# clearml/clearml-serving

Measured on AMD Instinct MI355X. Metric: requests/sec + p50 latency, ResNet-50 & BERT-base dyn-batch, 1/2/4/8 MI355X, higher is better.
Workload: dtype bf16; 1 GPU; model=resnet50+bert-base, global_batch=512, seq_len=128, image=3x224x224, parallelism=dp1, max_batch_size=64, outputs_consumed=16673280

## Files before the change

### clearml_serving_amd/models/resnet.py

```python

import torch
import torch.nn as nn
import torch.nn.functional as F

from .. import ops
from . import register_arch


class FoldedConv(nn.Module):

    def __init__(self, cin, cout, k, stride=1, padding=0, relu=False):
        super().__init__()
        self.conv = nn.Conv2d(cin, cout, k, stride=stride, padding=padding,
                              bias=True)
        self.relu = relu

    def forward(self, x):
        c = self.conv
        if (c.kernel_size == (3, 3) and c.stride == (1, 1)
                and c.padding == (1, 1)
                and ops.conv3x3_supported(x, c.weight)):
            return ops.conv3x3_nhwc(x, c.weight, c.bias, relu=self.relu)
        y = c(x)
        if self.relu:
            y = F.relu(y)
        return y


class StemConv(nn.Module):

    def __init__(self, cin, cout, k, stride, padding, relu=True):
        super().__init__()
        self.conv = nn.Conv2d(cin, cout, k, stride=stride, padding=padding,
                              bias=True)
        self.relu = relu
        self.k, self.stride, self.padding = k, stride, padding

    def forward(self, x):
        if not x.is_cuda:
            y = self.conv(x)
            return F.relu(y) if self.relu else y
        n, c, h, w = x.shape
        oh = (h + 2 * self.padding - self.k) // self.stride + 1
        ow = (w + 2 * self.padding - self.k) // self.stride + 1
        cols = F.unfold(x.contiguous(), self.k, stride=self.stride,
                        padding=self.padding)
        flat = cols.transpose(1, 2).reshape(-1, c * self.k * self.k)
        wmat = self.conv.weight.reshape(self.conv.out_channels, -1)
        y = torch.nn.functional.linear(flat, wmat, self.conv.bias)
        if self.relu:
            y = torch.relu(y)
        return y.view(n, oh, ow, self.conv.out_channels) \
            .permute(0, 3, 1, 2)


def fold_bn_into_conv(conv: nn.Conv2d, bn: nn.BatchNorm2d) -> None:
    with torch.no_grad():
        inv_std = torch.rsqrt(bn.running_var + bn.eps)
        scale = bn.weight * inv_std
        conv.weight.mul_(scale[:, None, None, None])
        bias = conv.bias.data if conv.bias is not None else torch.zeros_like(bn.bias)
        conv.bias = nn.Parameter(bn.bias + (bias - bn.running_mean) * scale)


class Bottleneck(nn.Module):
    expansion = 4

    def __init__(self, cin, width, stride=1, downsample=None):
        super().__init__()
        cout = width * self.expansion
        self.conv1 = FoldedConv(cin, width, 1, relu=True)
        self.conv2 = FoldedConv(width, width, 3, stride=stride, padding=1,
                                relu=True)
        self.conv3 = FoldedConv(width, cout, 1, relu=False)
        self.downsample = downsample

    def forward(self, x):
        identity = x if self.downsample is None else self.downsample(x)
        y = self.conv1(x)
        y = self.conv2(y)
        y = self.conv3.conv(y)
        return ops.bias_relu_add(y, residual=identity)


class ResNet(nn.Module):
    def __init__(self, layers=(3, 4, 6, 3), num_classes=1000):
        super().__init__()
        self.stem = FoldedConv(3, 64, 7, stride=2, padding=3, relu=True)
        self.maxpool = nn.MaxPool2d(3, stride=2, padding=1)
        self.inplanes = 64
        self.layer1 = self._make_layer(64, layers[0], stride=1)
        self.layer2 = self._make_layer(128, layers[1], stride=2)
        self.layer3 = self._make_layer(256, layers[2], stride=2)
        self.layer4 = self._make_layer(512, layers[3], stride=2)
        self.fc = nn.Linear(512 * Bottleneck.expansion, num_classes)
        self._init_weights()

    def _make_layer(self, width, blocks, stride):
        downsample = None
        cout = width * Bottleneck.expansion
        if stride != 1 or self.inplanes != cout:
            downsample = FoldedConv(self.inplanes, cout, 1, stride=stride)
        layers = [Bottleneck(self.inplanes, width, stride, downsample)]
        self.inplanes = cout
        for _ in range(1, blocks):
            layers.append(Bottleneck(self.inplanes, width))
        return nn.Sequential(*layers)

    def _init_weights(self):
        for m in self.modules():
            if isinstance(m, nn.Conv2d):
                nn.init.kaiming_normal_(m.weight, mode="fan_out",
                                        nonlinearity="relu")
                if m.bias is not None:
                    nn.init.zeros_(m.bias)

    def forward(self, x):
        x = x.contiguous(memory_format=torch.channels_last)
        x = self.stem(x)
        x = self.maxpool(x)
        x = self.layer1(x)
        x = self.layer2(x)
        x = self.layer3(x)
        x = self.layer4(x)
        x = x.mean(dim=(2, 3))
        return self.fc(x)


@register_arch("resnet50")
def resnet50(num_classes: int = 1000) -> ResNet:
    return ResNet(layers=(3, 4, 6, 3), num_classes=num_classes).to(
        memory_format=torch.channels_last)


@register_arch("resnet101")
def resnet101(num_classes: int = 1000) -> ResNet:
    return ResNet(layers=(3, 4, 23, 3), num_classes=num_classes).to(
        memory_format=torch.channels_last)
```

### clearml_serving_amd/ops/__init__.py

```python

import importlib.machinery
import importlib.util
import math
import os
from typing import Optional, Tuple

import torch

_ext = None
_ext_error: Optional[str] = None
_FORCE_EAGER = os.environ.get("CLEARML_SERVING_AMD_FORCE_EAGER") == "1"


def _try_load_ext() -> None:
    global _ext, _ext_error
    if _ext is not None or _ext_error is not None:
        return
    so_path = os.path.join(os.path.dirname(__file__), "_hip_ops.so")
    if not os.path.exists(so_path):
        _ext_error = "extension not built ({} missing)".format(so_path)
        return
    try:
        loader = importlib.machinery.ExtensionFileLoader("_hip_ops", so_path)
        spec = importlib.util.spec_from_loader("_hip_ops", loader)
        mod = importlib.util.module_from_spec(spec)
        loader.exec_module(mod)
        _ext = mod
    except Exception as ex:
        _ext_error = "failed loading {}: {}".format(so_path, ex)


_try_load_ext()


def has_extension() -> bool:
    return _ext is not None


def _require_ext(opname: str):
    if _FORCE_EAGER:
        return None
    if _ext is None:
        raise RuntimeError(
            "clearml_serving_amd HIP extension required for GPU op '{}' but "
            "not loaded: {}. Build it with __graft_entry__.build() "
            "(hipcc --offload-arch=gfx950).".format(opname, _ext_error)
        )
    return _ext


def extension_or_none():
    return _ext


def layernorm(
    x: torch.Tensor, weight: torch.Tensor, bias: torch.Tensor,
    eps: float = 1e-5, residual: Optional[torch.Tensor] = None,
) -> torch.Tensor:
    if x.is_cuda:
        ext = _require_ext("layernorm")
        if ext is not None:
            return ext.layernorm(x, weight, bias, eps, residual)
    if residual is not None:
        x = x + residual
    return torch.nn.functional.layer_norm(
        x.float(), (x.shape[-1],), weight.float(), bias.float(), eps
    ).to(x.dtype)


def rmsnorm(
    x: torch.Tensor, weight: torch.Tensor, eps: float = 1e-6,
    residual: Optional[torch.Tensor] = None,
) -> torch.Tensor:
    if x.is_cuda:
        ext = _require_ext("rmsnorm")
        if ext is not None:
            return ext.rmsnorm(x, weight, eps, residual)
    xf = x.float()
    if residual is not None:
        xf = xf + residual.float()
        residual.copy_(xf.to(residual.dtype))
    out = xf * torch.rsqrt(xf.pow(2).mean(-1, keepdim=True) + eps)
    return (out * weight.float()).to(x.dtype)


def bias_gelu(x: torch.Tensor, bias: Optional[torch.Tensor] = None) -> torch.Tensor:
    if x.is_cuda:
        ext = _require_ext("bias_gelu")
        if ext is not None:
            return ext.bias_gelu(x, bias)
    if bias is not None:
        x = x + bias
    return torch.nn.functional.gelu(x.float()).to(x.dtype)


def bias_relu_add(
    x: torch.Tensor, bias: Optional[torch.Tensor] = None,
    residual: Optional[torch.Tensor] = None,
) -> torch.Tensor:
    if x.is_cuda:
        ext = _require_ext("bias_relu_add")
        if ext is not None:
            return ext.bias_relu_add(x, bias, residual)
    if bias is not None:
        x = x + bias
    if residual is not None:
        x = x + residual
    return torch.relu(x)


def silu_mul(gate: torch.Tensor, up: torch.Tensor) -> torch.Tensor:
    if gate.is_cuda:
        ext = _require_ext("silu_mul")
        if ext is not None:
            return ext.silu_mul(gate, up)
    return (torch.nn.functional.silu(gate.float()) * up.float()).to(gate.dtype)


F8_MAX = 448.0


def _quant_fp8_ref(y: torch.Tensor):
    y2 = y.float().reshape(-1, y.shape[-1])
    amax = y2.abs().amax(dim=1).clamp(min=1e-8)
    scale = (amax / F8_MAX).to(torch.float32)
    q = (y2 / scale[:, None]).clamp(-F8_MAX, F8_MAX).to(torch.float8_e4m3fn)
    return q.view(torch.uint8), scale


def rmsnorm_fp8(x: torch.Tensor, weight: torch.Tensor, eps: float = 1e-6,
                residual: Optional[torch.Tensor] = None):
    if x.is_cuda:
        ext = _require_ext("rmsnorm_fp8")
        if ext is not None:
            out8, scales = ext.rmsnorm_fp8(x, weight, eps, residual)
            return out8, scales
    return _quant_fp8_ref(rmsnorm(x, weight, eps, residual=residual))


def silu_mul_fp8(gate: torch.Tensor, up: torch.Tensor):
    if gate.is_cuda:
        ext = _require_ext("silu_mul_fp8")
        if ext is not None:
            out8, scales = ext.silu_mul_fp8(gate, up)
            return out8, scales
    return _quant_fp8_ref(silu_mul(gate, up))


def quant_fp8(x: torch.Tensor):
    if x.is_cuda:
        ext = _require_ext("quant_fp8")
        if ext is not None:
            out8, scales = ext.quant_fp8(x)
            return out8, scales
    return _quant_fp8_ref(x)


def swizzle_fp8_weight(w8: torch.Tensor) -> torch.Tensor:
    n, k = w8.shape
    assert k % 64 == 0
    v = w8.view(torch.uint8).reshape(n, k // 64, 2, 4, 8)
    return v.permute(0, 1, 3, 2, 4).contiguous().reshape(n, k)


def unswizzle_fp8_weight(w8s: torch.Tensor) -> torch.Tensor:
    n, k = w8s.shape
    v = w8s.view(torch.uint8).reshape(n, k // 64, 4, 2, 8)
    return v.permute(0, 1, 3, 2, 4).contiguous().reshape(n, k)


def skinny_gemm_fp8(a8: torch.Tensor, a_scale: torch.Tensor,
                    w8: torch.Tensor, w_scale: torch.Tensor,
                    swizzled: bool = False) -> torch.Tensor:
    if a8.is_cuda:
        ext = _require_ext("skinny_gemm_fp8")
        if ext is not None:
            ws = w8 if swizzled else swizzle_fp8_weight(w8)
            return ext.skinny_gemm_fp8(
                a8.view(torch.uint8), a_scale, ws.view(torch.uint8), w_scale)
    if swizzled:
        w8 = unswizzle_fp8_weight(w8)
    a = a8.view(torch.float8_e4m3fn).float() * a_scale[:, None]
    w = w8.view(torch.float8_e4m3fn).float() * w_scale[:, None]
    return (a @ w.t()).to(torch.bfloat16)


def skinny_gemm_fp8_v2(a8: torch.Tensor, a_scale: torch.Tensor,
                       w8: torch.Tensor, w_scale: torch.Tensor
                       ) -> torch.Tensor:
    if a8.is_cuda:
        ext = _require_ext("skinny_gemm_fp8_v2")
        if ext is not None:
            return ext.skinny_gemm_fp8_v2(
                a8.view(torch.uint8), a_scale, w8.view(torch.uint8), w_scale)
    a = a8.view(torch.float8_e4m3fn).float() * a_scale[:, None]
    w = w8.view(torch.float8_e4m3fn).float() * w_scale[:, None]
    return (a @ w.t()).to(torch.bfloat16)


def conv3x3_supported(x: torch.Tensor, w: torch.Tensor) -> bool:
    return (x.is_cuda and x.dtype == torch.bfloat16 and x.dim() == 4
            and x.shape[2] == x.shape[3] and x.shape[2] in (56, 28, 14)
            and x.shape[1] % 32 == 0 and w.shape[0] % 64 == 0
            and w.shape[2] == 3 and w.shape[3] == 3
            and os.environ.get("CMLS_CONV3", "1") != "0"
            and _ext is not None)


def conv3x3_nhwc(x: torch.Tensor, w: torch.Tensor,
                 bias: Optional[torch.Tensor] = None, relu: bool = False,
                 residual: Optional[torch.Tensor] = None) -> torch.Tensor:
    if (x.is_cuda and x.dtype == torch.bfloat16
            and x.shape[2] == x.shape[3] and x.shape[2] in (56, 28, 14)
            and x.shape[1] % 32 == 0 and w.shape[0] % 64 == 0):
        ext = _require_ext("conv3x3_nhwc")
        if ext is not None:
            xc = x.contiguous(memory_format=torch.channels_last)
            wc = w.contiguous(memory_format=torch.channels_last)
            return ext.conv3x3_nhwc(xc, wc, bias, relu, residual)
    y = torch.nn.functional.conv2d(x.float(), w.float(),
                                   bias.float() if bias is not None else None,
                                   stride=1, padding=1)
    if residual is not None:
        y = y + residual.float()
    if relu:
        y = torch.relu(y)
    return y.to(x.dtype)


def softmax(x: torch.Tensor, dim: int = -1) -> torch.Tensor:
    if x.is_cuda and dim in (-1, x.dim() - 1):
        ext = _require_ext("softmax")
        if ext is not None:
            return ext.softmax_lastdim(x)
    return torch.softmax(x.float(), dim=dim).to(x.dtype)


def attention(
    q: torch.Tensor, k: torch.Tensor, v: torch.Tensor,
    causal: bool = False, scale: Optional[float] = None,
    seq_lens: Optional[torch.Tensor] = None,
    layout: str = "bhsd",
) -> torch.Tensor:
    if scale is None:
        scale = 1.0 / math.sqrt(q.shape[-1])
    bshd = layout == "bshd"
    if q.is_cuda:
        ext = _require_ext("attention")
        if ext is not None:
            return ext.attention_prefill(q, k, v, bool(causal), float(scale),
                                         seq_lens, bshd)
    if bshd:
        out = attention(q.permute(0, 2, 1, 3), k.permute(0, 2, 1, 3),
                        v.permute(0, 2, 1, 3), causal=causal, scale=scale,
                        seq_lens=seq_lens)
        return out.permute(0, 2, 1, 3).contiguous()
    qf, kf, vf = q.float(), k.float(), v.float()
    hq, hkv = q.shape[1], k.shape[1]
    if hkv != hq:
        rep = hq // hkv
        kf = kf.repeat_interleave(rep, dim=1)
        vf = vf.repeat_interleave(rep, dim=1)
    scores = torch.matmul(qf, kf.transpose(-1, -2)) * scale
    sq, sk = q.shape[2], k.shape[2]
    if causal:
        mask = torch.ones(sq, sk, dtype=torch.bool, device=q.device).tril(
            diagonal=sk - sq)
        scores = scores.masked_fill(~mask, float("-inf"))
    if seq_lens is not None:
        key_idx = torch.arange(sk, device=q.device)
        pad = key_idx[None, None, None, :] >= seq_lens[:, None, None, None]
        scores = scores.masked_fill(pad, float("-inf"))
    probs = torch.softmax(scores, dim=-1)
    return torch.matmul(probs, vf).to(q.dtype)


def _dequant_kv_cpu(cache: torch.Tensor, scale: torch.Tensor) -> torch.Tensor:
    f = cache.view(torch.float8_e4m3fn).float()
    return f * scale[..., None]


def attention_prefill_paged(
    q: torch.Tensor, k_cache: torch.Tensor, v_cache: torch.Tensor,
    block_table: torch.Tensor, kv_lens: torch.Tensor, q_lens: torch.Tensor,
    scale: Optional[float] = None,
    k_scale: Optional[torch.Tensor] = None,
    v_scale: Optional[torch.Tensor] = None,
) -> torch.Tensor:
    if scale is None:
        scale = 1.0 / math.sqrt(q.shape[-1])
    if q.is_cuda:
        ext = _require_ext("attention_prefill_paged")
        if ext is not None:
            return ext.attention_prefill_paged(
                q, k_cache, v_cache, block_table, kv_lens, q_lens,
                float(scale), k_scale, v_scale)
    if k_scale is not None:
        return attention_prefill_paged(
            q, _dequant_kv_cpu(k_cache, k_scale),
            _dequant_kv_cpu(v_cache, v_scale), block_table, kv_lens, q_lens,
            scale)
    b, sq, h, d = q.shape
    hkv = k_cache.shape[1]
    bs = k_cache.shape[2]
    out = torch.zeros_like(q)
    for i in range(b):
        n = int(kv_lens[i])
        ql = int(q_lens[i])
        nb = (n + bs - 1) // bs
        blocks = block_table[i, :nb].long()
        k = k_cache[blocks].float().permute(1, 0, 2, 3).reshape(
            hkv, nb * bs, d)[:, :n]
        v = v_cache[blocks].float().permute(1, 0, 2, 3).reshape(
            hkv, nb * bs, d)[:, :n]
        o = attention(
            q[i, :ql].permute(1, 0, 2)[None].float(),
            k[None], v[None], causal=True, scale=scale)
        out[i, :ql] = o[0].permute(1, 0, 2).to(q.dtype)
    return out


def attention_decode(
    q: torch.Tensor, k_cache: torch.Tensor, v_cache: torch.Tensor,
    block_table: torch.Tensor, seq_lens: torch.Tensor,
    scale: Optional[float] = None,
    k_scale: Optional[torch.Tensor] = None,
    v_scale: Optional[torch.Tensor] = None,
) -> torch.Tensor:
    if scale is None:
        scale = 1.0 / math.sqrt(q.shape[-1])
    if q.is_cuda:
        ext = _require_ext("attention_decode")
        if ext is not None:
            return ext.attention_decode(q, k_cache, v_cache, block_table,
                                        seq_lens, float(scale),
                                        k_scale, v_scale)
    if k_scale is not None:
        return attention_decode(
            q, _dequant_kv_cpu(k_cache, k_scale),
            _dequant_kv_cpu(v_cache, v_scale), block_table, seq_lens, scale)
    bsz, hq, d = q.shape
    hkv = k_cache.shape[1]
    block_size = k_cache.shape[2]
    rep = hq // hkv
    out = torch.empty_like(q, dtype=q.dtype)
    qf = q.float()
    for b in range(bsz):
        n = int(seq_lens[b])
        nblocks = (n + block_size - 1) // block_size
        blocks = block_table[b, :nblocks].long()
        k = k_cache[blocks].float()
        v = v_cache[blocks].float()
        k = k.permute(1, 0, 2, 3).reshape(hkv, nblocks * block_size, d)[:, :n]
        v = v.permute(1, 0, 2, 3).reshape(hkv, nblocks * block_size, d)[:, :n]
        if rep > 1:
            k = k.repeat_interleave(rep, dim=0)
            v = v.repeat_interleave(rep, dim=0)
        scores = torch.einsum("hd,hnd->hn", qf[b], k) * scale
        probs = torch.softmax(scores, dim=-1)
        out[b] = torch.einsum("hn,hnd->hd", probs, v).to(q.dtype)
    return out


def kv_cache_write(
    k_new: torch.Tensor, v_new: torch.Tensor, k_cache: torch.Tensor,
    v_cache: torch.Tensor, slot_mapping: torch.Tensor,
    k_scale: Optional[torch.Tensor] = None,
    v_scale: Optional[torch.Tensor] = None,
) -> None:
    if k_new.is_cuda:
        ext = _require_ext("kv_cache_write")
        if ext is not None:
            ext.kv_cache_write(k_new, v_new, k_cache, v_cache, slot_mapping,
                               k_scale, v_scale)
            return
    block_size = k_cache.shape[2]
    fp8 = k_scale is not None
    for t in range(k_new.shape[0]):
        slot = int(slot_mapping[t])
        if slot < 0:
            continue
        blk, off = slot // block_size, slot % block_size
        if fp8:
            for cache, scales, new in ((k_cache, k_scale, k_new),
                                       (v_cache, v_scale, v_new)):
                row = new[t].float()
                amax = row.abs().amax(dim=-1).clamp_min(1e-8)
                sc = torch.exp2(torch.ceil(torch.log2(amax / 448.0)))
                q8 = (row / sc[:, None]).to(torch.float8_e4m3fn)
                cache[blk, :, off] = q8.view(torch.uint8)
                scales[blk, :, off] = sc
        else:
            k_cache[blk, :, off] = k_new[t]
            v_cache[blk, :, off] = v_new[t]


def rope_inplace(
    q: torch.Tensor, k: torch.Tensor, positions: torch.Tensor,
    theta: float = 10000.0,
) -> Tuple[torch.Tensor, torch.Tensor]:
    if q.is_cuda:
        ext = _require_ext("rope")
        if ext is not None:
            ext.rope_inplace(q, k, positions, float(theta))
            return q, k
    d = q.shape[-1]
    half = d // 2
    inv_freq = 1.0 / (theta ** (torch.arange(half, dtype=torch.float32,
                                             device=q.device) / half))
    angles = positions.float()[:, None] * inv_freq[None, :]
    cos = angles.cos()[:, None, :]
    sin = angles.sin()[:, None, :]
    for t in (q, k):
        tf = t.float().clone()
        lo, hi = tf[..., :half], tf[..., half:]
        t[..., :half] = (lo * cos - hi * sin).to(t.dtype)
        t[..., half:] = (hi * cos + lo * sin).to(t.dtype)
    return q, k


def sample_top_k_top_p(
    logits: torch.Tensor, temperature: float = 1.0, top_k: int = 0,
    top_p: float = 1.0, generator: Optional[torch.Generator] = None,
) -> torch.Tensor:
    if temperature == 0.0:
        return logits.argmax(dim=-1)
    if logits.is_cuda:
        ext = _require_ext("sample")
        if ext is not None:
            seed = int(torch.randint(0, 2**31 - 1, (1,),
                                     generator=generator).item())
            return ext.sample_top_k_top_p(
                logits, float(temperature), int(top_k), float(top_p), seed)
    lf = logits.float() / temperature
    if top_k and top_k < lf.shape[-1]:
        kth = torch.topk(lf, top_k, dim=-1).values[..., -1:]
        lf = lf.masked_fill(lf < kth, float("-inf"))
    if top_p < 1.0:
        sorted_logits, idx = torch.sort(lf, descending=True, dim=-1)
        probs = torch.softmax(sorted_logits, dim=-1)
        cutoff = probs.cumsum(dim=-1) > top_p
        cutoff[..., 0] = False
        sorted_logits = sorted_logits.masked_fill(cutoff, float("-inf"))
        lf = torch.full_like(lf, float("-inf")).scatter(-1, idx, sorted_logits)
    probs = torch.softmax(lf, dim=-1)
    return torch.multinomial(probs, 1, generator=generator).squeeze(-1)


def gemm_bf16(a: torch.Tensor, b: torch.Tensor) -> torch.Tensor:
    if a.is_cuda:
        ext = _require_ext("gemm_bf16")
        if ext is not None:
            m, k = a.shape
            n = b.shape[0]
            pm, pn, pk = (-m) % 128, (-n) % 128, (-k) % 32
            if pm or pn or pk:
                a2 = torch.nn.functional.pad(a, (0, pk, 0, pm))
                b2 = torch.nn.functional.pad(b, (0, pk, 0, pn))
                return ext.gemm_bf16(a2.contiguous(),
                                     b2.contiguous())[:m, :n].contiguous()
            return ext.gemm_bf16(a.contiguous(), b.contiguous())
    return (a.float() @ b.float().T).to(a.dtype)


def skinny_linear(x: torch.Tensor, weight: torch.Tensor) -> torch.Tensor:
    if (x.is_cuda and x.dtype == torch.bfloat16 and x.dim() == 2
            and x.shape[1] % 32 == 0 and weight.shape[0] % 16 == 0
            and os.environ.get("CMLS_SKINNY", "1") != "0"):
        m, k = x.shape
        n = weight.shape[0]
        if ((1 <= m <= 16 and n <= 8192 and k <= 8192)
                or (m <= 2 and n <= 8192)):
            ext = _require_ext("skinny_gemm")
            if ext is not None:
                return ext.skinny_gemm(x.contiguous(), weight, 1)
    return torch.nn.functional.linear(x, weight)


def lora_shrink(x: torch.Tensor, a: torch.Tensor,
                idx: torch.Tensor) -> torch.Tensor:
    if x.is_cuda:
        ext = _require_ext("lora_shrink")
        if ext is not None:
            return ext.lora_shrink(x.contiguous(), a, idx)
    sel = a.float().index_select(0, idx.clamp(min=0).long())
    y = torch.bmm(sel, x.float().unsqueeze(-1)).squeeze(-1)
    return torch.where((idx >= 0).unsqueeze(-1), y, torch.zeros_like(y))


def lora_expand_add(y: torch.Tensor, b: torch.Tensor, idx: torch.Tensor,
                    out: torch.Tensor) -> torch.Tensor:
    if out.is_cuda:
        ext = _require_ext("lora_expand_add")
        if ext is not None:
            ext.lora_expand_add(y, b, idx, out)
            return out
    live = (idx >= 0).unsqueeze(-1)
    sel = b.float().index_select(0, idx.clamp(min=0).long())
    yf = torch.where(live, y.float(), torch.zeros_like(y, dtype=torch.float32))
    delta = torch.bmm(sel, yf.unsqueeze(-1)).squeeze(-1)
    out.copy_(torch.where(live, (out.float() + delta).to(out.dtype), out))
    return out


def _check_mask_args(logits: torch.Tensor, bank: torch.Tensor,
                     slot: torch.Tensor) -> None:
    if logits.dim() != 2:
        raise ValueError("logits must be [B, V]")
    if bank.dtype != torch.int32 or bank.dim() != 2 \
            or bank.shape[1] != (logits.shape[1] + 31) // 32:
        raise ValueError("bank must be int32 [S, ceil(V/32)]")
    if slot.dtype != torch.int32 or slot.dim() != 1 \
            or slot.shape[0] != logits.shape[0]:
        raise ValueError("slot must be int32 [B]")


def _unpack_token_bitmask(bank: torch.Tensor, slot: torch.Tensor,
                          vocab: int) -> torch.Tensor:
    rows = bank.index_select(0, slot.clamp(min=0).long())
    shifts = torch.arange(32, dtype=torch.int32, device=bank.device)
    bits = (rows.unsqueeze(-1) >> shifts) & 1
    allowed = bits.reshape(rows.shape[0], -1)[:, :vocab].bool()
    return allowed | (slot < 0).unsqueeze(-1)


def apply_token_bitmask(logits: torch.Tensor, bank: torch.Tensor,
                        slot: torch.Tensor) -> torch.Tensor:
    if logits.is_cuda:
        ext = _require_ext("apply_token_bitmask")
        if ext is not None:
            return ext.apply_token_bitmask(logits, bank, slot)
    _check_mask_args(logits, bank, slot)
    allowed = _unpack_token_bitmask(bank, slot, logits.shape[1])
    return logits.masked_fill(~allowed, float("-inf"))


def sample_token_bitmask(logits: torch.Tensor, bank: torch.Tensor,
                         slot: torch.Tensor, temperature: torch.Tensor,
                         seed: torch.Tensor) -> torch.Tensor:
    if logits.is_cuda:
        ext = _require_ext("sample_token_bitmask")
        if ext is not None:
            return ext.sample_token_bitmask(logits, bank, slot, temperature,
                                            seed)
    _check_mask_args(logits, bank, slot)
    allowed = _unpack_token_bitmask(bank, slot, logits.shape[1])
    masked = logits.float().masked_fill(~allowed, float("-inf"))
    out = masked.argmax(dim=-1)
    for i in range(logits.shape[0]):
        t = float(temperature[i])
        if t > 0.0 and bool(allowed[i].any()):
            gen = torch.Generator(device=logits.device)
            gen.manual_seed(int(seed[i]) & 0x7FFFFFFF)
            probs = torch.softmax(masked[i] / t, dim=-1)
            out[i] = torch.multinomial(probs, 1, generator=gen)[0]
    return torch.where(allowed.any(dim=-1), out, torch.full_like(out, -1))
```

### clearml_serving_amd/ops/csrc/bindings.cpp

```cpp
#include <torch/extension.h>

torch::Tensor bias_relu_add(torch::Tensor x, c10::optional<torch::Tensor> bias,
                            c10::optional<torch::Tensor> residual);
torch::Tensor bias_gelu(torch::Tensor x, c10::optional<torch::Tensor> bias);
torch::Tensor silu_mul(torch::Tensor gate, torch::Tensor up);
torch::Tensor layernorm(torch::Tensor x, torch::Tensor weight,
                        torch::Tensor bias, double eps,
                        c10::optional<torch::Tensor> residual);
torch::Tensor rmsnorm(torch::Tensor x, torch::Tensor weight, double eps,
                      c10::optional<torch::Tensor> residual);
torch::Tensor softmax_lastdim(torch::Tensor x);
torch::Tensor attention_prefill(torch::Tensor q, torch::Tensor k,
                                torch::Tensor v, bool causal, double scale,
                                c10::optional<torch::Tensor> seq_lens,
                                bool bshd);
torch::Tensor sample_top_k_top_p(torch::Tensor logits, double temperature,
                                 long top_k, double top_p, long seed);
torch::Tensor attention_decode(torch::Tensor q, torch::Tensor k_cache,
                               torch::Tensor v_cache,
                               torch::Tensor block_table,
                               torch::Tensor seq_lens, double scale,
                               c10::optional<torch::Tensor> k_scale,
                               c10::optional<torch::Tensor> v_scale);
void kv_cache_write(torch::Tensor knew, torch::Tensor vnew,
                    torch::Tensor k_cache, torch::Tensor v_cache,
                    torch::Tensor slot_mapping,
                    c10::optional<torch::Tensor> k_scale,
                    c10::optional<torch::Tensor> v_scale);
torch::Tensor gemm_bf16(torch::Tensor a, torch::Tensor b);
torch::Tensor skinny_gemm(torch::Tensor a, torch::Tensor w, int64_t variant);
torch::Tensor attention_prefill_paged(
    torch::Tensor q, torch::Tensor k_cache, torch::Tensor v_cache,
    torch::Tensor block_table, torch::Tensor kv_lens, torch::Tensor q_lens,
    double scale, c10::optional<torch::Tensor> k_scale,
    c10::optional<torch::Tensor> v_scale);
void rope_inplace(torch::Tensor q, torch::Tensor k, torch::Tensor positions,
                  double theta);
std::vector<torch::Tensor> rmsnorm_fp8(torch::Tensor x, torch::Tensor weight,
                                       double eps,
                                       c10::optional<torch::Tensor> residual);
std::vector<torch::Tensor> silu_mul_fp8(torch::Tensor gate, torch::Tensor up);
std::vector<torch::Tensor> quant_fp8(torch::Tensor x);
torch::Tensor skinny_gemm_fp8(torch::Tensor a8, torch::Tensor a_scale,
                              torch::Tensor w8, torch::Tensor w_scale);
torch::Tensor skinny_gemm_fp8_v2(torch::Tensor a8, torch::Tensor a_scale,
                                 torch::Tensor w8, torch::Tensor w_scale);
torch::Tensor conv3x3_nhwc(torch::Tensor x, torch::Tensor w,
                           c10::optional<torch::Tensor> bias, bool relu,
                           c10::optional<torch::Tensor> residual);
torch::Tensor lora_shrink(torch::Tensor x, torch::Tensor a, torch::Tensor idx);
void lora_expand_add(torch::Tensor y, torch::Tensor b, torch::Tensor idx,
                     torch::Tensor out);
torch::Tensor apply_token_bitmask(torch::Tensor logits, torch::Tensor bank,
                                  torch::Tensor slot);
torch::Tensor sample_token_bitmask(torch::Tensor logits, torch::Tensor bank,
                                   torch::Tensor slot,
                                   torch::Tensor temperature,
                                   torch::Tensor seed);

PYBIND11_MODULE(TORCH_EXTENSION_NAME, m) {
  m.doc() = "clearml-serving-amd gfx950 kernel library";
  m.def("bias_relu_add", &bias_relu_add, py::arg("x"),
        py::arg("bias") = py::none(), py::arg("residual") = py::none());
  m.def("bias_gelu", &bias_gelu, py::arg("x"), py::arg("bias") = py::none());
  m.def("silu_mul", &silu_mul);
  m.def("layernorm", &layernorm, py::arg("x"), py::arg("weight"),
        py::arg("bias"), py::arg("eps") = 1e-5,
        py::arg("residual") = py::none());
  m.def("rmsnorm", &rmsnorm, py::arg("x"), py::arg("weight"),
        py::arg("eps") = 1e-6, py::arg("residual") = py::none());
  m.def("softmax_lastdim", &softmax_lastdim);
  m.def("attention_prefill", &attention_prefill, py::arg("q"), py::arg("k"),
        py::arg("v"), py::arg("causal"), py::arg("scale"),
        py::arg("seq_lens") = py::none(), py::arg("bshd") = false);
  m.def("sample_top_k_top_p", &sample_top_k_top_p);
  m.def("rope_inplace", &rope_inplace);
  m.def("attention_decode", &attention_decode, py::arg("q"),
        py::arg("k_cache"), py::arg("v_cache"), py::arg("block_table"),
        py::arg("seq_lens"), py::arg("scale"),
        py::arg("k_scale") = py::none(), py::arg("v_scale") = py::none());
  m.def("kv_cache_write", &kv_cache_write, py::arg("knew"), py::arg("vnew"),
        py::arg("k_cache"), py::arg("v_cache"), py::arg("slot_mapping"),
        py::arg("k_scale") = py::none(), py::arg("v_scale") = py::none());
  m.def("gemm_bf16", &gemm_bf16);
  m.def("skinny_gemm", &skinny_gemm, py::arg("a"), py::arg("w"),
        py::arg("variant") = 0);
  m.def("attention_prefill_paged", &attention_prefill_paged, py::arg("q"),
        py::arg("k_cache"), py::arg("v_cache"), py::arg("block_table"),
        py::arg("kv_lens"), py::arg("q_lens"), py::arg("scale"),
        py::arg("k_scale") = py::none(), py::arg("v_scale") = py::none());
  m.def("rmsnorm_fp8", &rmsnorm_fp8, py::arg("x"), py::arg("weight"),
        py::arg("eps") = 1e-6, py::arg("residual") = py::none());
  m.def("silu_mul_fp8", &silu_mul_fp8);
  m.def("quant_fp8", &quant_fp8);
  m.def("skinny_gemm_fp8", &skinny_gemm_fp8);
  m.def("skinny_gemm_fp8_v2", &skinny_gemm_fp8_v2);
  m.def("conv3x3_nhwc", &conv3x3_nhwc, py::arg("x"), py::arg("w"),
        py::arg("bias") = py::none(), py::arg("relu") = false,
        py::arg("residual") = py::none());
  m.def("lora_shrink", &lora_shrink, py::arg("x"), py::arg("a"),
        py::arg("idx"));
  m.def("lora_expand_add", &lora_expand_add, py::arg("y"), py::arg("b"),
        py::arg("idx"), py::arg("out"));
  m.def("apply_token_bitmask", &apply_token_bitmask, py::arg("logits"),
        py::arg("bank"), py::arg("slot"));
  m.def("sample_token_bitmask", &sample_token_bitmask, py::arg("logits"),
        py::arg("bank"), py::arg("slot"), py::arg("temperature"),
        py::arg("seed"));
}
```

Before: 11070 requests/s.

## Add fused MFMA conv1x1 NHWC kernel with bias, ReLU and residual epilogue

Adds a custom HIP conv1x1 kernel for channels-last bf16 activations, implemented as an MFMA GEMM with double-buffered LDS staging via global_load_lds and an XCD-aware tile remap. It is used for stride-1 1x1 convs in the ResNet bottlenecks. For conv3 the bias, residual add and ReLU are fused into the GEMM epilogue, which removes the separate bias_relu_add pass and the round trip of its intermediate tensor through memory. The risk is that this hand-written GEMM may be slower than the vendor library for some shapes. Inputs with Cin >= 2048 and strided 1x1 convs still use the old path.

Measured after the change: 12560 requests/s, median of 5. 1.13x the previous value.

```diff
diff --git a/clearml_serving_amd/models/resnet.py b/clearml_serving_amd/models/resnet.py
--- a/clearml_serving_amd/models/resnet.py
+++ b/clearml_serving_amd/models/resnet.py
@@ -17,6 +17,10 @@
 
     def forward(self, x):
         c = self.conv
+        if (c.kernel_size == (1, 1) and c.stride == (1, 1)
+                and c.padding == (0, 0) and c.groups == 1
+                and ops.conv1x1_supported(x, c.weight)):
+            return ops.conv1x1_nhwc(x, c.weight, c.bias, relu=self.relu)
         if (c.kernel_size == (3, 3) and c.stride == (1, 1)
                 and c.padding == (1, 1)
                 and ops.conv3x3_supported(x, c.weight)):
@@ -79,7 +83,11 @@
         identity = x if self.downsample is None else self.downsample(x)
         y = self.conv1(x)
         y = self.conv2(y)
-        y = self.conv3.conv(y)
+        c3 = self.conv3.conv
+        if ops.conv1x1_supported(y, c3.weight):
+            return ops.conv1x1_nhwc(y, c3.weight, c3.bias, relu=True,
+                                    residual=identity)
+        y = c3(y)
         return ops.bias_relu_add(y, residual=identity)
 
 
diff --git a/clearml_serving_amd/ops/__init__.py b/clearml_serving_amd/ops/__init__.py
--- a/clearml_serving_amd/ops/__init__.py
+++ b/clearml_serving_amd/ops/__init__.py
@@ -221,6 +221,47 @@
     y = torch.nn.functional.conv2d(x.float(), w.float(),
                                    bias.float() if bias is not None else None,
                                    stride=1, padding=1)
+    if residual is not None:
+        y = y + residual.float()
+    if relu:
+        y = torch.relu(y)
+    return y.to(x.dtype)
+
+
+def _has_nhwc_strides(t: torch.Tensor) -> bool:
+    n, c, h, w = t.shape
+    sn, sc, sh, sw = t.stride()
+    return ((c == 1 or sc == 1) and (w == 1 or sw == c)
+            and (h == 1 or sh == w * c) and (n == 1 or sn == h * w * c))
+
+
+def conv1x1_supported(x: torch.Tensor, w: torch.Tensor) -> bool:
+    return (x.is_cuda and x.dtype == torch.bfloat16 and x.dim() == 4
+            and x.shape[1] < 2048
+            and w.dim() == 4 and w.dtype == torch.bfloat16
+            and w.shape[2] == 1 and w.shape[3] == 1
+            and w.shape[1] == x.shape[1]
+            and x.shape[1] % 32 == 0 and w.shape[0] % 64 == 0
+            and x.numel() > 0
+            and _has_nhwc_strides(x)
+            and w.stride(0) == w.shape[1] and w.stride(1) == 1
+            and os.environ.get("CMLS_CONV1", "1") != "0"
+            and _ext is not None)
+
+
+def conv1x1_nhwc(x: torch.Tensor, w: torch.Tensor,
+                 bias: Optional[torch.Tensor] = None, relu: bool = False,
+                 residual: Optional[torch.Tensor] = None) -> torch.Tensor:
+    if conv1x1_supported(x, w):
+        if residual is not None and not (
+                residual.dtype == x.dtype and _has_nhwc_strides(residual)):
+            residual = residual.to(x.dtype).contiguous(
+                memory_format=torch.channels_last)
+        return _ext.conv1x1_nhwc(x, w, bias, relu, residual)
+    if x.is_cuda:
+        _require_ext("conv1x1_nhwc")
+    y = torch.nn.functional.conv2d(x.float(), w.float(),
+                                   bias.float() if bias is not None else None)
     if residual is not None:
         y = y + residual.float()
     if relu:
diff --git a/clearml_serving_amd/ops/csrc/bindings.cpp b/clearml_serving_amd/ops/csrc/bindings.cpp
--- a/clearml_serving_amd/ops/csrc/bindings.cpp
+++ b/clearml_serving_amd/ops/csrc/bindings.cpp
@@ -46,6 +46,9 @@
 torch::Tensor skinny_gemm_fp8_v2(torch::Tensor a8, torch::Tensor a_scale,
                                  torch::Tensor w8, torch::Tensor w_scale);
 torch::Tensor conv3x3_nhwc(torch::Tensor x, torch::Tensor w,
+                           c10::optional<torch::Tensor> bias, bool relu,
+                           c10::optional<torch::Tensor> residual);
+torch::Tensor conv1x1_nhwc(torch::Tensor x, torch::Tensor w,
                            c10::optional<torch::Tensor> bias, bool relu,
                            c10::optional<torch::Tensor> residual);
 torch::Tensor lora_shrink(torch::Tensor x, torch::Tensor a, torch::Tensor idx);
@@ -98,6 +101,9 @@
   m.def("conv3x3_nhwc", &conv3x3_nhwc, py::arg("x"), py::arg("w"),
         py::arg("bias") = py::none(), py::arg("relu") = false,
         py::arg("residual") = py::none());
+  m.def("conv1x1_nhwc", &conv1x1_nhwc, py::arg("x"), py::arg("w"),
+        py::arg("bias") = py::none(), py::arg("relu") = false,
+        py::arg("residual") = py::none());
   m.def("lora_shrink", &lora_shrink, py::arg("x"), py::arg("a"),
         py::arg("idx"));
   m.def("lora_expand_add", &lora_expand_add, py::arg("y"), py::arg("b"),
diff --git a/clearml_serving_amd/ops/csrc/conv1x1.hip b/clearml_serving_amd/ops/csrc/conv1x1.hip
--- /dev/null
+++ b/clearml_serving_amd/ops/csrc/conv1x1.hip
@@ -0,0 +1,256 @@
+#include "common.h"
+
+namespace {
+
+typedef __attribute__((ext_vector_type(8))) short bf16x8_t;
+typedef __attribute__((ext_vector_type(4))) float f32x4_t;
+
+#define MFMA_16x16x32(A, B, C) \
+  __builtin_amdgcn_mfma_f32_16x16x32_bf16((A), (B), (C), 0, 0, 0)
+
+constexpr int BM = 128, BK = 32;
+
+__device__ __forceinline__ int swz_group(int row, int g) {
+  return g ^ ((row >> 2) & 3);
+}
+
+__device__ __forceinline__ int chan_of_lds_row(int l) {
+  const int j = l >> 4, i = l & 15;
+  return (j >> 1) * 32 + (i >> 2) * 8 + (j & 1) * 4 + (i & 3);
+}
+
+template <int BN, bool RELU, bool HAS_RES>
+__global__ __launch_bounds__(256, 2) void conv1x1_kernel(
+    const __hip_bfloat16* __restrict__ A,
+    const __hip_bfloat16* __restrict__ B,
+    const __hip_bfloat16* __restrict__ bias,
+    const __hip_bfloat16* __restrict__ res,
+    __hip_bfloat16* __restrict__ C,
+    int M, int N, int K) {
+  constexpr int WN = BN / 2;
+  constexpr int NF = WN / 16;
+  constexpr int NH = NF / 2;
+  __shared__ short lds_a[2][BM * BK];
+  __shared__ short lds_b[2][BN * BK];
+
+  const int tiles_n = N / BN;
+  const int nwg = gridDim.x;
+  const int xcd = blockIdx.x % 8;
+  const int idx = blockIdx.x / 8;
+  const int q8 = nwg / 8, r8 = nwg % 8;
+  const int bid = (xcd < r8 ? xcd * (q8 + 1)
+                            : r8 * (q8 + 1) + (xcd - r8) * q8) + idx;
+  const int bm = bid / tiles_n;
+  const int bn = bid % tiles_n;
+
+  const int tid = threadIdx.x;
+  const int lane = tid & 63;
+  const int wave = tid >> 6;
+  const int wm = (wave >> 1) * 64;
+  const int wn = (wave & 1) * WN;
+
+  const int frag_i = lane & 15;
+  const int frag_g = lane >> 4;
+
+  const int st_row = tid >> 2;
+  const int st_g = tid & 3;
+
+  const __hip_bfloat16* a_src[2];
+#pragma unroll
+  for (int half = 0; half < 2; ++half) {
+    const int row = st_row + half * 64;
+    const int grow = min(bm * BM + row, M - 1);
+    a_src[half] = A + (long)grow * K + swz_group(row, st_g) * 8;
+  }
+  const __hip_bfloat16* b_src[BN / 64];
+#pragma unroll
+  for (int half = 0; half < BN / 64; ++half) {
+    const int row = st_row + half * 64;
+    const int n = bn * BN + (row / WN) * WN + chan_of_lds_row(row % WN);
+    b_src[half] = B + (long)n * K + swz_group(row, st_g) * 8;
+  }
+
+  auto stage = [&](int buf, int kt) {
+    const int k0 = kt * BK;
+#pragma unroll
+    for (int half = 0; half < 2; ++half) {
+      const int row = st_row + half * 64;
+      short* dst = &lds_a[buf][row * BK + st_g * 8];
+      __builtin_amdgcn_global_load_lds(
+          reinterpret_cast<const unsigned int*>(a_src[half] + k0),
+          reinterpret_cast<unsigned int*>(dst), 16, 0, 0);
+    }
+#pragma unroll
+    for (int half = 0; half < BN / 64; ++half) {
+      const int row = st_row + half * 64;
+      short* dst = &lds_b[buf][row * BK + st_g * 8];
+      __builtin_amdgcn_global_load_lds(
+          reinterpret_cast<const unsigned int*>(b_src[half] + k0),
+          reinterpret_cast<unsigned int*>(dst), 16, 0, 0);
+    }
+  };
+
+  f32x4_t acc[4][NF];
+#pragma unroll
+  for (int i = 0; i < 4; ++i)
+#pragma unroll
+    for (int j = 0; j < NF; ++j) acc[i][j] = f32x4_t{0.f, 0.f, 0.f, 0.f};
+
+  const int ntiles = K / BK;
+  stage(0, 0);
+  asm volatile("s_waitcnt vmcnt(0)" ::: "memory");
+  __syncthreads();
+
+  for (int kt = 0; kt < ntiles; ++kt) {
+    const int cur = kt & 1;
+    if (kt + 1 < ntiles) stage(cur ^ 1, kt + 1);
+
+    bf16x8_t a_frag[4], b_frag[NF];
+#pragma unroll
+    for (int m = 0; m < 4; ++m) {
+      const int row = wm + m * 16 + frag_i;
+      a_frag[m] = *reinterpret_cast<const bf16x8_t*>(
+          &lds_a[cur][row * BK + swz_group(row, frag_g) * 8]);
+    }
+#pragma unroll
+    for (int n = 0; n < NF; ++n) {
+      const int row = wn + n * 16 + frag_i;
+      b_frag[n] = *reinterpret_cast<const bf16x8_t*>(
+          &lds_b[cur][row * BK + swz_group(row, frag_g) * 8]);
+    }
+    __builtin_amdgcn_s_setprio(1);
+#pragma unroll
+    for (int m = 0; m < 4; ++m)
+#pragma unroll
+      for (int n = 0; n < NF; ++n)
+        acc[m][n] = MFMA_16x16x32(b_frag[n], a_frag[m], acc[m][n]);
+    __builtin_amdgcn_s_setprio(0);
+
+    asm volatile("s_waitcnt vmcnt(0)" ::: "memory");
+    __syncthreads();
+  }
+
+  const int g = lane >> 4;
+  const int ccol0 = bn * BN + wn + g * 8;
+  float bv[NH][8];
+#pragma unroll
+  for (int h = 0; h < NH; ++h) {
+    if (bias) {
+      bf16x8 b8;
+      b8.u = *reinterpret_cast<const uint32x4*>(bias + ccol0 + h * 32);
+#pragma unroll
+      for (int e = 0; e < 8; ++e) bv[h][e] = to_f32(b8.h[e]);
+    } else {
+#pragma unroll
+      for (int e = 0; e < 8; ++e) bv[h][e] = 0.f;
+    }
+  }
+#pragma unroll
+  for (int m = 0; m < 4; ++m) {
+    const int row = bm * BM + wm + m * 16 + (lane & 15);
+    const long off = (long)min(row, M - 1) * N + ccol0;
+    bf16x8 r8v[NH];
+    if (HAS_RES) {
+#pragma unroll
+      for (int h = 0; h < NH; ++h)
+        r8v[h].u = *reinterpret_cast<const uint32x4*>(res + off + h * 32);
+    }
+#pragma unroll
+    for (int h = 0; h < NH; ++h) {
+      bf16x8 o8;
+#pragma unroll
+      for (int e = 0; e < 8; ++e) {
+        float v = acc[m][2 * h + (e >> 2)][e & 3] + bv[h][e];
+        if (HAS_RES) v += to_f32(r8v[h].h[e]);
+        if (RELU) v = fmaxf(v, 0.f);
+        o8.h[e] = __float2bfloat16(v);
+      }
+      if (row < M)
+        *reinterpret_cast<uint32x4*>(C + off + h * 32) = o8.u;
+    }
+  }
+}
+
+}
+
+#ifndef CMLS_KERNEL_ONLY
+torch::Tensor conv1x1_nhwc(torch::Tensor x, torch::Tensor w,
+                           c10::optional<torch::Tensor> bias, bool relu,
+                           c10::optional<torch::Tensor> residual) {
+  TORCH_CHECK(x.dim() == 4 && w.dim() == 4, "conv1x1: 4-D tensors");
+  TORCH_CHECK(x.is_cuda() && w.is_cuda(), "conv1x1: GPU tensors");
+  TORCH_CHECK(x.scalar_type() == at::kBFloat16 &&
+              w.scalar_type() == at::kBFloat16, "conv1x1: bf16 only");
+  const long Nb = x.size(0), Cin = x.size(1), H = x.size(2), W = x.size(3);
+  const long Cout = w.size(0);
+  TORCH_CHECK(w.size(1) == Cin && w.size(2) == 1 && w.size(3) == 1,
+              "conv1x1: weight must be [K, C, 1, 1]");
+  auto nhwc = [](const torch::Tensor& t, long c, long h, long wd) {
+    return (t.size(1) == 1 || t.stride(1) == 1) &&
+           (t.size(3) == 1 || t.stride(3) == c) &&
+           (t.size(2) == 1 || t.stride(2) == wd * c) &&
+           (t.size(0) == 1 || t.stride(0) == h * wd * c);
+  };
+  TORCH_CHECK(nhwc(x, Cin, H, W), "conv1x1: x must have NHWC strides");
+  TORCH_CHECK(w.stride(0) == Cin && (Cin == 1 || w.stride(1) == 1),
+              "conv1x1: weight must be [K, C] contiguous");
+  TORCH_CHECK(Cin % BK == 0, "conv1x1: Cin % 32 != 0");
+  TORCH_CHECK(Cout % 64 == 0, "conv1x1: Cout % 64 != 0");
+  const long M = Nb * H * W;
+  TORCH_CHECK(M >= 1 && M * std::max(Cin, Cout) < (1L << 40),
+              "conv1x1: empty or oversized input");
+  TORCH_CHECK(M < (1L << 31) - BM, "conv1x1: M too large");
+
+  auto out = torch::empty_strided(
+      {Nb, Cout, H, W}, {H * W * Cout, 1, W * Cout, Cout}, x.options());
+  const __hip_bfloat16* bp = nullptr;
+  if (bias.has_value() && bias->defined()) {
+    TORCH_CHECK(bias->scalar_type() == at::kBFloat16 && bias->is_cuda() &&
+                bias->is_contiguous() && bias->numel() == Cout,
+                "conv1x1: bias must be contiguous bf16 [K]");
+    bp = (const __hip_bfloat16*)bias->data_ptr();
+  }
+  const __hip_bfloat16* rp = nullptr;
+  if (residual.has_value() && residual->defined()) {
+    TORCH_CHECK(residual->scalar_type() == at::kBFloat16 &&
+                residual->is_cuda() && residual->sizes() == out.sizes() &&
+                nhwc(*residual, Cout, H, W),
+                "conv1x1: residual must be bf16 [N, K, H, W] with NHWC "
+                "strides");
+    rp = (const __hip_bfloat16*)residual->data_ptr();
+  }
+  auto aligned16 = [](const void* p) {
+    return reinterpret_cast<uintptr_t>(p) % 16 == 0;
+  };
+  TORCH_CHECK(aligned16(x.data_ptr()) && aligned16(w.data_ptr()) &&
+              aligned16(bp) && aligned16(rp),
+              "conv1x1: operands must be 16-byte aligned");
+  const int BN = (Cout % 128 == 0) ? 128 : 64;
+  const long tiles = ((M + BM - 1) / BM) * (Cout / BN);
+  TORCH_CHECK(tiles < (1L << 31), "conv1x1: grid too large");
+  dim3 grid((unsigned)tiles);
+  hipStream_t stream_ = cmls::current_stream();
+
+#define LAUNCH_C1(BN_, RELU_, RES_)                                         \
+  hipLaunchKernelGGL((conv1x1_kernel<BN_, RELU_, RES_>), grid, dim3(256),  \
+                     0, stream_, (const __hip_bfloat16*)x.data_ptr(),       \
+                     (const __hip_bfloat16*)w.data_ptr(), bp, rp,           \
+                     (__hip_bfloat16*)out.data_ptr(), (int)M, (int)Cout,    \
+                     (int)Cin)
+#define LAUNCH_C1_BN(BN_)                                                   \
+  do {                                                                      \
+    if (rp) {                                                               \
+      if (relu) LAUNCH_C1(BN_, true, true);                                 \
+      else LAUNCH_C1(BN_, false, true);                                     \
+    } else {                                                                \
+      if (relu) LAUNCH_C1(BN_, true, false);                                \
+      else LAUNCH_C1(BN_, false, false);                                    \
+    }                                                                       \
+  } while (0)
+  if (BN == 128) LAUNCH_C1_BN(128);
+  else LAUNCH_C1_BN(64);
+#undef LAUNCH_C1_BN
+#undef LAUNCH_C1
+  return out;
+}
+#endif
```
